# jambo6/online-neural-cdes

Measured on AMD Instinct MI355X. Metric: solved integration steps/sec (fwd+adjoint), higher is better.
Workload: dtype f32; 1 GPU; BASELINE cfg2: rectilinear interpolation, rk4 step 1, B=4096 per GPU (global 4096), raw L=200 -> T=399 knots, C=20, H=HH=32, nl=3; step = forward + adjoint backward + Adam; global_batch=4096, seq_len=200, parallelism=dp1

## Files before the change

### include/ncde_hip.h

```cpp
#ifndef NCDE_HIP_H
#define NCDE_HIP_H

#include <stddef.h>
#include <stdint.h>

#ifdef __cplusplus
extern "C" {
#endif

#define NCDE_ABI_VERSION 4
#define NCDE_MAX_LAYERS 8

typedef enum NcdeStatus {
    NCDE_OK = 0,
    NCDE_ERR_INVALID = -1,
    NCDE_ERR_UNSUPPORTED = -2,
    NCDE_ERR_WORKSPACE = -3,
    NCDE_ERR_HIP = -4
} NcdeStatus;

typedef enum NcdeInterp { NCDE_INTERP_LINEAR = 0, NCDE_INTERP_CUBIC = 1, NCDE_INTERP_QUINTIC = 2 } NcdeInterp;

typedef enum NcdeMethod { NCDE_EULER = 0, NCDE_MIDPOINT = 1, NCDE_RK4_38 = 2 } NcdeMethod;

typedef enum NcdeOutput { NCDE_OUT_INTERVAL = 0, NCDE_OUT_KNOTS = 1, NCDE_OUT_TIMES = 2 } NcdeOutput;

#define NCDE_FLAG_AUTO 0u
#define NCDE_FLAG_FORCE_GENERIC 1u
#define NCDE_FLAG_FORCE_FAST 2u
#define NCDE_FLAG_FP32_MFMA 4u
#define NCDE_FLAG_ADJOINT_V1 8u
#define NCDE_FLAG_ADJOINT_V2 16u
#define NCDE_FLAG_ADJOINT_V4 32u
#define NCDE_FLAG_SPLIT_BF16 64u
#define NCDE_FLAG_ADJOINT_SPLIT_FP16 128u
#define NCDE_FLAG_DEBUG_PROFILE 0x100u
#define NCDE_FLAG_NO_COOP 0x400u
#define NCDE_FLAG_COOP_FAULT_INJECT 0x800u
#define NCDE_FLAG_TILED_NS1 0x1000u
#define NCDE_FLAG_TILED_NS2 0x2000u
#define NCDE_FLAG_TILED_NS4 0x4000u
#define NCDE_FLAG_FORCE_TILED 0x8000u

#define NCDE_FLAG_TILED_WINDOW_STEPS(n) (((uint32_t)(n) & 0xFFu) << 16)

typedef struct NcdeProblem {
    int32_t abi_version;
    int32_t batch;
    int32_t n_knots;
    int32_t channels;
    int32_t hidden;
    int32_t interp;
    int32_t method;
    int32_t output;
    uint32_t flags;

    int32_t n_layers;
    int32_t layer_in[NCDE_MAX_LAYERS];
    int32_t layer_out[NCDE_MAX_LAYERS];
    const float* layer_W[NCDE_MAX_LAYERS];
    const float* layer_b[NCDE_MAX_LAYERS];
    const float* Wo;
    const float* bo;

    const float* coeffs;
    int64_t coeffs_stride_b;
    int64_t coeffs_stride_t;

    const float* z0;

    int32_t field_kind;
    int32_t field_input;
    const float* Wg;
    const float* bg;
    const float* Wr;
    const float* br;

    const void* time_plan;
    int32_t n_t_out;
    int32_t n_steps_fwd;
    int32_t n_steps_adj;
    int32_t reserved_;
} NcdeProblem;

typedef enum NcdeFieldKind { NCDE_FIELD_ORIGINAL = 0, NCDE_FIELD_MINIMAL = 1, NCDE_FIELD_GRU = 2 } NcdeFieldKind;
typedef enum NcdeFieldInput { NCDE_INPUT_MATMUL = 0, NCDE_INPUT_EVALUATE = 1, NCDE_INPUT_DERIVATIVE = 2 } NcdeFieldInput;

typedef struct NcdeGrads {
    float* grad_z0;
    float* grad_layer_W[NCDE_MAX_LAYERS];
    float* grad_layer_b[NCDE_MAX_LAYERS];
    float* grad_Wo;
    float* grad_bo;
    float* grad_Wg;
    float* grad_bg;
    float* grad_Wr;
    float* grad_br;
} NcdeGrads;

typedef struct NcdeTimeSpec {
    int32_t n_t;
    int32_t time_is_f64;
    const double* t;
    double step_size;
    const double* knots;
} NcdeTimeSpec;

typedef struct NcdeTimePlanInfo {
    int32_t n_t_out;
    int32_t n_steps_fwd;
    int32_t n_steps_adj;
    int32_t stages;
    int64_t bytes;
} NcdeTimePlanInfo;

int ncde_time_plan_build(const NcdeProblem* p, const NcdeTimeSpec* ts, void* host_buffer, size_t bytes, NcdeTimePlanInfo* info);

typedef struct NcdeAdaptiveOptions {
    double rtol, atol;
    double min_step;
    double max_step;
    double first_step;
    double safety, ifactor, dfactor;
    int32_t max_num_steps;
    int32_t trace_capacity;
    double* trace;
    int32_t replay_count;
    int32_t reserved_;
    const double* replay;
} NcdeAdaptiveOptions;

typedef struct NcdeAdaptiveStats {
    int32_t nfe;
    int32_t n_accepted, n_rejected;
    int32_t reserved_;
} NcdeAdaptiveStats;

int64_t ncde_dopri5_workspace_bytes(const NcdeProblem* p, const NcdeTimeSpec* ts, int pass );
const char* ncde_dopri5_kernel_name(const NcdeProblem* p, int pass );
int ncde_dopri5_forward(const NcdeProblem* p, const NcdeTimeSpec* ts, const NcdeAdaptiveOptions* opt, float* out, void* workspace,
                        size_t workspace_bytes, void* stream, NcdeAdaptiveStats* stats);
int ncde_dopri5_adjoint(const NcdeProblem* p, const NcdeTimeSpec* ts, const NcdeAdaptiveOptions* opt, const float* z_out,
                        const float* grad_out, const NcdeGrads* grads, void* workspace, size_t workspace_bytes, void* stream,
                        NcdeAdaptiveStats* stats);

int64_t ncde_dopri5_record_bytes(const NcdeProblem* p, const NcdeTimeSpec* ts, const NcdeAdaptiveOptions* opt);
int ncde_dopri5_forward_record(const NcdeProblem* p, const NcdeTimeSpec* ts, const NcdeAdaptiveOptions* opt, float* out, void* record,
                               size_t record_bytes, void* workspace, size_t workspace_bytes, void* stream, NcdeAdaptiveStats* stats);
int ncde_dopri5_backward(const NcdeProblem* p, const NcdeTimeSpec* ts, const NcdeAdaptiveOptions* opt, const void* record,
                         size_t record_bytes, const float* grad_out, const NcdeGrads* grads, void* workspace, size_t workspace_bytes,
                         void* stream);

int ncde_version(void);
const char* ncde_last_error_string(void);

int ncde_num_outputs(const NcdeProblem* p);

int64_t ncde_workspace_bytes(const NcdeProblem* p, int pass);

int64_t ncde_coop_status_offset(const NcdeProblem* p, int pass);

const char* ncde_kernel_name(const NcdeProblem* p, int pass);

int ncde_forward(const NcdeProblem* p, float* out, void* workspace, size_t workspace_bytes, void* stream);

int ncde_adjoint(const NcdeProblem* p, const float* z_out, const float* grad_out, const NcdeGrads* grads,
                 void* workspace, size_t workspace_bytes, void* stream);

int64_t ncde_stage_record_bytes(const NcdeProblem* p);
int ncde_forward_record(const NcdeProblem* p, float* out, float* stages, void* workspace, size_t workspace_bytes, void* stream);
int ncde_backward(const NcdeProblem* p, const float* stages, const float* grad_out, const NcdeGrads* grads, void* workspace,
                  size_t workspace_bytes, void* stream);

int64_t ncde_control_workspace_bytes(const NcdeProblem* p);
const char* ncde_control_kernel_name(const NcdeProblem* p);
int ncde_backward_control(const NcdeProblem* p, const float* stages, const float* grad_out, const NcdeGrads* grads, float* grad_coeffs,
                          void* workspace, size_t workspace_bytes, void* stream);

int ncde_time_kernel(const NcdeProblem* p, int pass, float* out, const float* grad_out, const NcdeGrads* grads,
                     void* workspace, size_t workspace_bytes, void* stream, int iters, float* ms_per_launch);

int64_t ncde_prepare_workspace_bytes(int kind, int B, int L, int C);
int ncde_prepare_linear(const float* x, int B, int L, int C, int rectilinear_time_index, float* out, void* stream);
int ncde_prepare_cubic(const float* x, int B, int L, int C, float* out, void* workspace, size_t workspace_bytes, void* stream);
int ncde_prepare_linear_grid(const float* x, const float* t, int B, int L, int C, int rectilinear_time_index, float* out, void* stream);
int ncde_prepare_cubic_grid(const float* x, const float* t, int B, int L, int C, float* out, void* workspace, size_t workspace_bytes, void* stream);
const char* ncde_prepare_kernel_name(int kind, int B, int L, int C, int has_grid, int rectilinear_time_index);


int ncde_smooth_pieces(int T, double eps);
int ncde_prepare_smooth(const float* x, int B, int T, int C, double eps, int order, float* out, void* stream);

#ifdef __cplusplus
}
#endif
// ... 2 lines not shown
```

### online-neural-cdes_amd/_lib.py

```python
import ctypes
import os

NCDE_ABI_VERSION = 4
NCDE_MAX_LAYERS = 8

INTERP = {"linear": 0, "cubic": 1, "quintic": 2}
INTERP_PARTS = {"linear": 1, "cubic": 4, "quintic": 6}
METHOD = {"euler": 0, "midpoint": 1, "rk4": 2}
OUT_INTERVAL, OUT_KNOTS, OUT_TIMES = 0, 1, 2
FIELD_KIND = {"original": 0, "minimal": 1, "gru": 2}
FIELD_INPUT = {"matmul": 0, "evaluate": 1, "derivative": 2}
FLAG_AUTO, FLAG_FORCE_GENERIC, FLAG_FORCE_FAST, FLAG_FP32_MFMA, FLAG_ADJOINT_V1, FLAG_ADJOINT_V2 = 0, 1, 2, 4, 8, 16
FLAG_ADJOINT_V4 = 32
FLAG_SPLIT_BF16 = 64
FLAG_NO_COOP = 0x400
FLAG_COOP_FAULT_INJECT = 0x800
FLAG_ADJOINT_SPLIT_FP16 = 128


def FLAG_TILED_WINDOW_STEPS(n):
    return (int(n) & 0xFF) << 16
FLAG_TILED_NS1, FLAG_TILED_NS2, FLAG_TILED_NS4, FLAG_FORCE_TILED = 0x1000, 0x2000, 0x4000, 0x8000

_c_float_p = ctypes.c_void_p


class NcdeProblem(ctypes.Structure):
    _fields_ = [
        ("abi_version", ctypes.c_int32),
        ("batch", ctypes.c_int32),
        ("n_knots", ctypes.c_int32),
        ("channels", ctypes.c_int32),
        ("hidden", ctypes.c_int32),
        ("interp", ctypes.c_int32),
        ("method", ctypes.c_int32),
        ("output", ctypes.c_int32),
        ("flags", ctypes.c_uint32),
        ("n_layers", ctypes.c_int32),
        ("layer_in", ctypes.c_int32 * NCDE_MAX_LAYERS),
        ("layer_out", ctypes.c_int32 * NCDE_MAX_LAYERS),
        ("layer_W", _c_float_p * NCDE_MAX_LAYERS),
        ("layer_b", _c_float_p * NCDE_MAX_LAYERS),
        ("Wo", _c_float_p),
        ("bo", _c_float_p),
        ("coeffs", _c_float_p),
        ("coeffs_stride_b", ctypes.c_int64),
        ("coeffs_stride_t", ctypes.c_int64),
        ("z0", _c_float_p),
        ("field_kind", ctypes.c_int32),
        ("field_input", ctypes.c_int32),
        ("Wg", _c_float_p),
        ("bg", _c_float_p),
        ("Wr", _c_float_p),
        ("br", _c_float_p),
        ("time_plan", ctypes.c_void_p),
        ("n_t_out", ctypes.c_int32),
        ("n_steps_fwd", ctypes.c_int32),
        ("n_steps_adj", ctypes.c_int32),
        ("reserved_", ctypes.c_int32),
    ]


class NcdeTimeSpec(ctypes.Structure):
    _fields_ = [
        ("n_t", ctypes.c_int32),
        ("time_is_f64", ctypes.c_int32),
        ("t", ctypes.POINTER(ctypes.c_double)),
        ("step_size", ctypes.c_double),
        ("knots", ctypes.POINTER(ctypes.c_double)),
    ]


class NcdeTimePlanInfo(ctypes.Structure):
    _fields_ = [
        ("n_t_out", ctypes.c_int32),
        ("n_steps_fwd", ctypes.c_int32),
        ("n_steps_adj", ctypes.c_int32),
        ("stages", ctypes.c_int32),
        ("bytes", ctypes.c_int64),
    ]


class NcdeAdaptiveOptions(ctypes.Structure):
    _fields_ = [(n, ctypes.c_double) for n in ("rtol", "atol", "min_step", "max_step", "first_step", "safety", "ifactor", "dfactor")] + \
               [("max_num_steps", ctypes.c_int32), ("trace_capacity", ctypes.c_int32), ("trace", ctypes.POINTER(ctypes.c_double)),
                ("replay_count", ctypes.c_int32), ("reserved_", ctypes.c_int32), ("replay", ctypes.POINTER(ctypes.c_double))]


class NcdeAdaptiveStats(ctypes.Structure):
    _fields_ = [("nfe", ctypes.c_int32), ("n_accepted", ctypes.c_int32), ("n_rejected", ctypes.c_int32), ("reserved_", ctypes.c_int32)]


class NcdeGrads(ctypes.Structure):
    _fields_ = [
        ("grad_z0", _c_float_p),
        ("grad_layer_W", _c_float_p * NCDE_MAX_LAYERS),
        ("grad_layer_b", _c_float_p * NCDE_MAX_LAYERS),
        ("grad_Wo", _c_float_p),
        ("grad_bo", _c_float_p),
        ("grad_Wg", _c_float_p),
        ("grad_bg", _c_float_p),
        ("grad_Wr", _c_float_p),
        ("grad_br", _c_float_p),
    ]


EXPORTS = (
    "ncde_version", "ncde_last_error_string", "ncde_num_outputs", "ncde_workspace_bytes",
    "ncde_kernel_name", "ncde_forward", "ncde_adjoint", "ncde_time_kernel",
    "ncde_prepare_workspace_bytes", "ncde_prepare_linear", "ncde_prepare_cubic", "ncde_prepare_linear_grid", "ncde_prepare_cubic_grid",
    "ncde_prepare_kernel_name",
    "ncde_smooth_pieces", "ncde_prepare_smooth",
    "ncde_stage_record_bytes", "ncde_forward_record", "ncde_backward",
    "ncde_time_plan_build", "ncde_dopri5_workspace_bytes", "ncde_dopri5_forward", "ncde_dopri5_adjoint",
    "ncde_dopri5_record_bytes", "ncde_dopri5_forward_record", "ncde_dopri5_backward", "ncde_dopri5_kernel_name",
    "ncde_coop_status_offset",
    "ncde_control_workspace_bytes", "ncde_control_kernel_name", "ncde_backward_control",
)

_LIB = None
LIB_PATH = os.path.join(os.path.dirname(os.path.abspath(__file__)), "libncde_hip.so")


class NcdeError(RuntimeError):
    pass


def source_fingerprint():
    import glob
    import hashlib
    here = os.path.dirname(os.path.abspath(__file__))
    files = sorted(glob.glob(os.path.join(here, "csrc", "*.hip")) + glob.glob(os.path.join(here, "csrc", "*.h")))
    files.append(os.path.join(os.path.dirname(here), "include", "ncde_hip.h"))
    h = hashlib.sha256()
    for f in files:
        h.update(os.path.basename(f).encode())
        with open(f, "rb") as fh:
            h.update(fh.read())
    return h.hexdigest()


def lib():
    global _LIB
    if _LIB is not None:
        return _LIB
    if not os.path.exists(LIB_PATH):
        raise NcdeError(
            "libncde_hip.so is not built (%s). Run `python __graft_entry__.py` or "
            "`make -C online-neural-cdes_amd/csrc`; there is no CPU fallback." % LIB_PATH)
    h = ctypes.CDLL(LIB_PATH)
    P = ctypes.POINTER(NcdeProblem)
    G = ctypes.POINTER(NcdeGrads)
    vp, sz = ctypes.c_void_p, ctypes.c_size_t
    h.ncde_version.restype = ctypes.c_int
    h.ncde_last_error_string.restype = ctypes.c_char_p
    h.ncde_num_outputs.argtypes = [P]
    h.ncde_num_outputs.restype = ctypes.c_int
    h.ncde_workspace_bytes.argtypes = [P, ctypes.c_int]
    h.ncde_workspace_bytes.restype = ctypes.c_int64
    h.ncde_coop_status_offset.argtypes = [P, ctypes.c_int]
    h.ncde_coop_status_offset.restype = ctypes.c_int64
    h.ncde_kernel_name.argtypes = [P, ctypes.c_int]
    h.ncde_kernel_name.restype = ctypes.c_char_p
    h.ncde_forward.argtypes = [P, vp, vp, sz, vp]
    h.ncde_forward.restype = ctypes.c_int
    h.ncde_adjoint.argtypes = [P, vp, vp, G, vp, sz, vp]
    h.ncde_adjoint.restype = ctypes.c_int
    h.ncde_time_kernel.argtypes = [P, ctypes.c_int, vp, vp, G, vp, sz, vp, ctypes.c_int, ctypes.POINTER(ctypes.c_float)]
    h.ncde_time_kernel.restype = ctypes.c_int
    h.ncde_stage_record_bytes.argtypes = [P]
# ... 61 lines not shown
```

### online-neural-cdes_amd/csrc/ncde_common.h

```cpp
#pragma once
#include <hip/hip_runtime.h>
#include <stdint.h>

#include "ncde_hip.h"

typedef float f32x4 __attribute__((ext_vector_type(4)));

__device__ __forceinline__ float quintic_eval(const float* p, int cs, float f, bool value) {
    const float bb = p[cs], c2 = p[2 * cs], d3 = p[3 * cs], e4 = p[4 * cs], f5 = p[5 * cs];
    if (value) {
        float inner = 0.25f * e4 + (f5 * f) / 5.0f;
        inner = d3 / 3.0f + inner * f;
        inner = 0.5f * c2 + inner * f;
        inner = bb + inner * f;
        return p[0] + inner * f;
    }
    float inner = e4 + f5 * f;
    inner = d3 + inner * f;
    inner = c2 + inner * f;
    return bb + inner * f;
}

#define NCDE_TILE 16

struct KArgs {
    int B, T, C, H, interp, method, output, n_layers, n_pieces, n_out;
    int din[NCDE_MAX_LAYERS], dout[NCDE_MAX_LAYERS];
    const float* W[NCDE_MAX_LAYERS];
    const float* b[NCDE_MAX_LAYERS];
    const float* Wo;
    const float* bo;
    const float* coeffs;
    long long cs_b, cs_t;
    const float* z0;
    float* out;
    const float* z_out;
    const float* grad_out;
    float* grad_z0;
    float* gpart;
    int gW_off[NCDE_MAX_LAYERS], gb_off[NCDE_MAX_LAYERS];
    int gWo_off, gbo_off, theta_size;
    int gacc_in_lds;
    float* stages;
    int discrete;
    float* recA;
    float* recB;
    float* recC;
    float* recD;
    int gstride;
    int win_hi, win_lo, resume;
    float* carry;
    int field_kind, field_input;
    int d0;
    int rows;
    const float* Wg;
    const float* bg;
    const float* Wr;
    const float* br;
    int gWg_off, gbg_off, gWr_off, gbr_off;
    const int* plan;
    int n_steps_fwd, n_steps_adj;
    const float* Wo_pk;
    int* fault;
    int only_faulted;
    const float* Wg_pk;
    const unsigned* Wo_bf;
    int wres[NCDE_MAX_LAYERS], wres_o, wres_g, wres_r;
    int tres[NCDE_MAX_LAYERS], tres_o, tres_g;
    int Hr, Cc;
    const unsigned* coop_img;
    float* coop_x;
    float* coop_state;
    unsigned* coop_sync;
    const float* coop_scale;
    int coop_M, coop_G;
    float* recS;
    unsigned* win_max;
    int dw2_parts;
    int dw2_accum;
    int Brec;
    unsigned* coop_status;
    const unsigned* run_if;
    unsigned coop_spin;
    int coop_inject;
};

typedef void (*NcdeKernel)(KArgs);

#define NCDE_PLAN_MAGIC 0x4e43504c
#define NCDE_PLAN_HEADER 8
struct StageDesc {
    int idx;
    float frac;
    float kdt;
};
__host__ __device__ __forceinline__ int plan_step_words(int S) { return 3 + 3 * S; }
__host__ __device__ __forceinline__ int plan_off_fwd() { return NCDE_PLAN_HEADER; }
__host__ __device__ __forceinline__ int plan_off_out(int S, int n_fwd) { return NCDE_PLAN_HEADER + n_fwd * plan_step_words(S); }
__host__ __device__ __forceinline__ int plan_off_adj(int S, int n_fwd, int n_out) { return plan_off_out(S, n_fwd) + 2 * n_out; }
__device__ __forceinline__ bool plan_header_ok(const KArgs& a, int S) {
    const int* h = a.plan;
    return h[0] == NCDE_PLAN_MAGIC && h[1] == S && h[2] == a.n_steps_fwd && h[3] == a.n_steps_adj && h[4] == a.n_out;
}
__device__ __forceinline__ StageDesc plan_stage(const int* step, int j) {
    StageDesc d;
    d.idx = step[3 + 3 * j];
    d.frac = __int_as_float(step[4 + 3 * j]);
    d.kdt = __int_as_float(step[5 + 3 * j]);
    return d;
}

__device__ __forceinline__ int ru4(int x) { return (x + 3) & ~3; }
__device__ __forceinline__ int ru16(int x) { return (x + 15) & ~15; }

__device__ __forceinline__ f32x4 mfma16(float a, float b, f32x4 c) {
    return __builtin_amdgcn_mfma_f32_16x16x4f32(a, b, c, 0, 0, 0);
}

__device__ __forceinline__ float tanh_dev(float x) {
    const float e = __builtin_amdgcn_exp2f(x * 2.8853900817779268f);
    const float r = __builtin_amdgcn_rcpf(e + 1.0f);
    return __builtin_fmaf(-2.0f, r, 1.0f);
}

#define NCDE_TANH_PRESCALE 2.8853900817779268f
__device__ __forceinline__ float tanh_prescaled(float x2l) {
    const float e = __builtin_amdgcn_exp2f(x2l);
    const float r = __builtin_amdgcn_rcpf(e + 1.0f);
    return __builtin_fmaf(-2.0f, r, 1.0f);
}

__device__ __forceinline__ float relu_dev(float x) { return __builtin_amdgcn_fmed3f(x, 0.0f, __builtin_inff()); }

__device__ __forceinline__ int n_stages(int method) { return method == NCDE_RK4_38 ? 4 : (method == NCDE_MIDPOINT ? 2 : 1); }
__device__ __forceinline__ float stage_offset(int method, int j) {
    if (method == NCDE_RK4_38) return j == 0 ? 0.0f : (j == 1 ? 0.333333343267440796f : (j == 2 ? 0.666666686534881592f : 1.0f));
    if (method == NCDE_MIDPOINT) return j == 0 ? 0.0f : 0.5f;
    return 0.0f;
}
__device__ __forceinline__ float stage_weight(int method, int j) {
    if (method == NCDE_RK4_38) return (j == 0 || j == 3) ? 0.125f : 0.375f;
    if (method == NCDE_MIDPOINT) return j == 0 ? 0.0f : 1.0f;
    return 1.0f;
}

__device__ __forceinline__ int piece_index(float t, int n_pieces) {
    int idx = (int)__builtin_ceilf(t) - 1;
    idx = idx < 0 ? 0 : idx;
    return idx > n_pieces - 1 ? n_pieces - 1 : idx;
}

__device__ __forceinline__ float row16_sum(float v) {
    v += __shfl_xor(v, 8, 64);
    v += __shfl_xor(v, 4, 64);
    v += __shfl_xor(v, 2, 64);
    v += __shfl_xor(v, 1, 64);
    return v;
}

struct StageCombine {
    __device__ static __forceinline__ float apply(int method, int j, float k, float dt, float& y0, float& k1, float& k2, bool& last) {
        last = false;
        if (method == NCDE_RK4_38) {
            if (j == 0) { k1 = k; return y0 + (dt * k) * 0.333333343267440796f; }
            if (j == 1) { k2 = k; return y0 + dt * (k - k1 * 0.333333343267440796f); }
            if (j == 2) { const float ys = y0 + dt * ((k1 - k2) + k); k2 = k2 + k; return ys; }
            last = true;
            y0 = y0 + (((k1 + 3.0f * k2) + k) * dt) * 0.125f;
            return y0;
        }
        if (method == NCDE_MIDPOINT) {
            if (j == 0) return y0 + k * (0.5f * dt);
            last = true;
            y0 = y0 + dt * k;
            return y0;
        }
        last = true;
        y0 = y0 + dt * k;
        return y0;
    }
};

__device__ __forceinline__ StageDesc default_stage(int method, float t, int n_pieces) {
    StageDesc d;
    d.idx = piece_index(t, n_pieces);
    d.frac = t - (float)d.idx;
    d.kdt = 1.0f;
    return d;
}

__device__ __forceinline__ float plan_out_cotangent(const KArgs& a, const int* pstep, const int* pout, int part, long long brow, int h) {
    float acc = 0.0f;
    const int q0 = pstep[1], q1 = q0 + pstep[2];
    for (int q = q0; q < q1; ++q) {
        const int kind = pout[2 * q];
        const float slope = __int_as_float(pout[2 * q + 1]);
        const float g = a.grad_out[(brow + q) * a.Hr + h];
        if (part == 1) acc += kind == 1 ? g : (kind == 2 ? slope * g : 0.0f);
        else acc += kind == 0 ? g : (kind == 2 ? g - slope * g : 0.0f);
    }
    return acc;
}
```

### online-neural-cdes_amd/csrc/ncde_fast.hip

```cpp
#include "ncde_fast.h"
#include "ncde_fast4.h"
#include "ncde_fast64.h"
#include "ncde_fast_nl.h"
#include "ncde_fast_c.h"
#include "ncde_fast_fwd3.h"
#include "ncde_fast_plan.h"
#ifndef NCDE_F2_DW_LATE
#define NCDE_F2_DW_LATE 0
#endif
#ifndef NCDE_F2_DXL_BF3
#define NCDE_F2_DXL_BF3 1
#endif
#ifndef NCDE_F2_DWO_EARLY
#define NCDE_F2_DWO_EARLY 0
#endif
#ifndef NCDE_H2_DW_LATE
#define NCDE_H2_DW_LATE 1
#endif
#ifndef NCDE_H2_DWO_EARLY
#define NCDE_H2_DWO_EARLY 0
#endif

#include <cstring>
#include <type_traits>
// ... 115 lines not shown

    const int n_inner = a.n_layers - 1;
    int zpar = 0;
    if constexpr (PROF != 0) tlast = __builtin_readcyclecounter();
    for (int n = 0; n < a.T - 1; ++n) {
        if (n + 1 < a.n_pieces) stage_load(n + 1);
#pragma unroll
        for (int j = 0; j < S; ++j) {
            const float t = (float)n + stage_offset(METHOD, j);
            const int idx = piece_index(t, a.n_pieces);
            const float frac = t - (float)idx;
            const float* dxp = dxs[idx % 3] + s * DXW;
            if (a.stages != nullptr && wave == ((n * S + j) % NW) && valid) {
                float* rec = a.stages + ((long long)(n * S + j) * a.B + bs) * a.Hr;
#pragma unroll
                for (int ks = 0; ks < HB; ++ks)
                    if (4 * ks + g < a.Hr) rec[4 * ks + g] = zreg[ks];
            }
            f32x4 acc[HT];
            float hB[KH];
#pragma unroll
            for (int tt = 0; tt < HT; ++tt) acc[tt] = bias0[tt];
#pragma unroll
            for (int ks = 0; ks < HB; ++ks)
#pragma unroll
                for (int tt = 0; tt < HT; ++tt) acc[tt] = mfma16(w0[tt][ks], zreg[ks], acc[tt]);
#pragma unroll
            for (int tt = 0; tt < HT; ++tt)
#pragma unroll
                for (int r = 0; r < 4; ++r) hB[4 * tt + r] = relu_dev(acc[tt][r]);
            for (int rep = 0; rep < n_inner; ++rep) {
#pragma unroll
                for (int tt = 0; tt < HT; ++tt) acc[tt] = bias1[tt];
#pragma unroll
                for (int ks = 0; ks < KH; ++ks)
#pragma unroll
                    for (int tt = 0; tt < HT; ++tt) acc[tt] = mfma16(w1[tt][ks], hB[ks], acc[tt]);
#pragma unroll
                for (int tt = 0; tt < HT; ++tt)
#pragma unroll
                    for (int r = 0; r < 4; ++r) hB[4 * tt + r] = relu_dev(acc[tt][r]);
            }
            NCDE_TICK(0)
            float kout[NB];
#pragma unroll
            for (int nb = 0; nb < NB; ++nb) kout[nb] = 0.0f;
            f32x4 oprev[NB];
#pragma unroll
            for (int cq = 0; cq <= CQ; ++cq) {
                f32x4 o[NB];
                if (cq < CQ) {
#pragma unroll
                    for (int nb = 0; nb < NB; ++nb) o[nb] = biaso[nb][cq];
#pragma unroll
                    for (int ks = 0; ks < KH; ++ks)
#pragma unroll
                        for (int nb = 0; nb < NB; ++nb) o[nb] = mfma16(wo[nb][cq][ks], hB[ks], o[nb]);
                }
                if (cq > 0) {
                    const int cp = cq - 1;
                    f32x4 dx;
                    if constexpr (INTERP == NCDE_INTERP_LINEAR) {
                        dx = *reinterpret_cast<const f32x4*>(dxp + 4 * cp);
                    } else {
                        const f32x4 cb = *reinterpret_cast<const f32x4*>(dxp + 4 * cp);
                        const f32x4 cc = *reinterpret_cast<const f32x4*>(dxp + CP + 4 * cp);
                        const f32x4 cd = *reinterpret_cast<const f32x4*>(dxp + 2 * CP + 4 * cp);
#pragma unroll
                        for (int r = 0; r < 4; ++r) {
                            const float inner = cc[r] + cd[r] * frac;
                            dx[r] = cb[r] + inner * frac;
                        }
                    }
#pragma unroll
                    for (int nb = 0; nb < NB; ++nb)
#pragma unroll
                        for (int r = 0; r < 4; ++r) kout[nb] = fmaf(tanh_prescaled(oprev[nb][r]), dx[r], kout[nb]);
                }
                if (cq > 0 && cq < CQ) {
#pragma unroll
                    for (int i = 0; i < KH * NB; ++i) {
                        __builtin_amdgcn_sched_group_barrier(0x008, 1, 0);
                        __builtin_amdgcn_sched_group_barrier(0x002, 3, 0);
                    }
                }
#pragma unroll
                for (int nb = 0; nb < NB; ++nb) oprev[nb] = o[nb];
            }
            NCDE_TICK(1)
            float ys[NB];
#pragma unroll
            for (int nb = 0; nb < NB; ++nb) ys[nb] = Combine<METHOD>::apply(j, kout[nb], y0[nb], k1[nb], k2[nb]);
            if (j == S - 1) {
                if (valid && (a.output == NCDE_OUT_KNOTS || n == a.T - 2)) {
                    const int row = a.output == NCDE_OUT_KNOTS ? n + 1 : 1;
#pragma unroll
                    for (int nb = 0; nb < NB; ++nb)
                        if (4 * (wave * NB + nb) + g < a.Hr) a.out[((long long)bs * a.n_out + row) * a.Hr + 4 * (wave * NB + nb) + g] = ys[nb];
                }
                if (n + 1 < a.n_pieces) stage_store(n + 1);
            }
            if constexpr (NW == 1) {
#pragma unroll
                for (int nb = 0; nb < NB; ++nb) zreg[nb] = ys[nb];
                __builtin_amdgcn_fence(__ATOMIC_RELEASE, "wavefront");
            } else {
                float* zw = zx[zpar];
#pragma unroll
                for (int nb = 0; nb < NB; ++nb) zw[(4 * (wave * NB + nb) + g) * 16 + s] = ys[nb];
                __syncthreads();
#pragma unroll
                for (int ks = 0; ks < HB; ++ks) zreg[ks] = zw[(4 * ks + g) * 16 + s];
                zpar ^= 1;
            }
            NCDE_TICK(2)
        }
    }
    if constexpr (PROF != 0) {
        if (lane == 0) {
            unsigned long long* dst = reinterpret_cast<unsigned long long*>(a.gpart) + ((long long)blockIdx.x * NW + wave) * 4;
            dst[0] = prof[0]; dst[1] = prof[1]; dst[2] = prof[2]; dst[3] = prof[3];
        }
    }
#undef NCDE_TICK
}

template <int H, int HH, int C, int NW, int INTERP, int METHOD, int PROF = 0, int NLT = 0, int HP = 0, int PLAN = 0>
__global__ __launch_bounds__(64 * NW, (NW + 3) / 4) void ncde_fwd_fast_bf3(KArgs a) {
    unsigned long long prof[4] = {0, 0, 0, 0}, tlast = 0;
#define NCDE_TICK(k)                                                \
    if constexpr (PROF != 0) {                                      \
        const unsigned long long now_ = __builtin_readcyclecounter(); \
        prof[k] += now_ - tlast;                                    \
        tlast = now_;                                               \
    }
    constexpr int CP = (C + 3) & ~3, CQ = CP / 4, HB = H / 4, HT = HH / 16, NB = HB / NW;
    constexpr int KC0 = H / 32, KC = HH / 32;
    constexpr int S = kStages<METHOD>;
    constexpr int NT = 64 * NW;
    constexpr int DXW = INTERP == NCDE_INTERP_LINEAR ? CP : 3 * CP;
    constexpr int EPT = (16 * DXW + NT - 1) / NT;
    static_assert(H % (4 * NW) == 0 && HH % 32 == 0 && H % 32 == 0, "shape not tileable");
    __shared__ __attribute__((aligned(16))) float zx[2][H * 16];
    __shared__ __attribute__((aligned(16))) float dxs[PLAN ? 1 : 3][PLAN ? 4 : 16 * DXW];
    __shared__ __attribute__((aligned(16))) float dxq[PLAN ? 2 : 1][PLAN ? S * 16 * CP : 4];
    __shared__ int fault_s;
    if constexpr (HP == 0) {
        if (a.only_faulted && a.fault[blockIdx.x] == 0) return;
    }
    if constexpr (PLAN != 0) {
        if (a.plan == nullptr || !plan_header_ok(a, S)) return;
    }
    float mx = 0.0f;

    const int tid = threadIdx.x, lane = tid & 63;
    const int wave = __builtin_amdgcn_readfirstlane(tid >> 6);
    const int s = lane & 15, g = lane >> 4;
    const int b0 = blockIdx.x * NCDE_TILE;
    const int bs = b0 + s;
    const bool valid = bs < a.B;

    typedef SplitOps<HP> SO;
    typedef typename SO::T SpT;
    SpT w0[HT][KC0], w1[HT][KC], wo[NB][CQ][KC];
    f32x4 bias0[HT], bias1[HT], biaso[NB][CQ];
    const bool has_inner = a.n_layers > 1;
#pragma unroll
    for (int t = 0; t < HT; ++t) {
        const int unitA = 32 * (t >> 1) + 8 * (s >> 2) + 4 * (t & 1) + (s & 3);
        float tmp[8];
#pragma unroll
        for (int c = 0; c < KC0; ++c) {
#pragma unroll
            for (int j = 0; j < 8; ++j) tmp[j] = a.W[0][unitA * H + 32 * c + 8 * g + j];
            w0[t][c] = SO::split(tmp, mx);
        }
#pragma unroll
        for (int c = 0; c < KC; ++c) {
#pragma unroll
            for (int j = 0; j < 8; ++j) tmp[j] = has_inner ? a.W[1][unitA * HH + 32 * c + 8 * g + j] : 0.0f;
            w1[t][c] = SO::split(tmp, mx);
        }
#pragma unroll
        for (int r = 0; r < 4; ++r) {
            const int unitD = 32 * (t >> 1) + 8 * g + 4 * (t & 1) + r;
            bias0[t][r] = a.b[0][unitD];
            bias1[t][r] = has_inner ? a.b[1][unitD] : 0.0f;
        }
    }
#pragma unroll
    for (int nb = 0; nb < NB; ++nb) {
        const int hb = wave * NB + nb;
#pragma unroll
        for (int cq = 0; cq < CQ; ++cq) {
            const int hA = 4 * hb + (s >> 2), cA = 4 * cq + (s & 3);
            float tmp[8];
#pragma unroll
            for (int c = 0; c < KC; ++c) {
#pragma unroll
                for (int j = 0; j < 8; ++j) tmp[j] = cA < C ? NCDE_TANH_PRESCALE * a.Wo[(hA * C + cA) * HH + 32 * c + 8 * g + j] : 0.0f;
                wo[nb][cq][c] = SO::split(tmp, mx);
            }
#pragma unroll
            for (int r = 0; r < 4; ++r) {
                const int cc = 4 * cq + r;
                biaso[nb][cq][r] = cc < C ? NCDE_TANH_PRESCALE * a.bo[(4 * hb + g) * C + cc] : 0.0f;
            }
        }
    }

    const float* eptr[EPT];
    float eprev[EPT], enext[EPT];
    bool eok[EPT];
#pragma unroll
    for (int q = 0; q < EPT; ++q) {
        const int e = tid + q * NT;
        const int es = e / DXW, ec = e - es * DXW;
        const int part = ec / CP, c = ec - part * CP;
        eok[q] = e < 16 * DXW && c < a.Cc && (b0 + es) < a.B;
        const long long base = (long long)(eok[q] ? b0 + es : 0) * a.cs_b;
        eptr[q] = a.coeffs + base + (INTERP == NCDE_INTERP_LINEAR ? c : (part + 1) * a.Cc + c);
        eprev[q] = 0.0f;
        enext[q] = 0.0f;
    }
    auto stage_load = [&](int piece) {
#pragma unroll
        for (int q = 0; q < EPT; ++q) {
            const int row = INTERP == NCDE_INTERP_LINEAR ? piece + 1 : piece;
            enext[q] = eok[q] ? eptr[q][(long long)row * a.cs_t] : 0.0f;
        }
    };
    auto stage_store = [&](int piece) {
        float* dst = dxs[piece % 3];
#pragma unroll
        for (int q = 0; q < EPT; ++q) {
            const int e = tid + q * NT;
            if (e < 16 * DXW) dst[e] = INTERP == NCDE_INTERP_LINEAR ? enext[q] - eprev[q] : enext[q];
            eprev[q] = enext[q];
        }
    };
    constexpr int EPQ = PLAN ? (S * 16 * CP + NT - 1) / NT : 1;
    float qn[EPQ];
    auto plan_load = [&](const int* pstep) {
#pragma unroll
        for (int q = 0; q < EPQ; ++q) {
            const int e = tid + q * NT;
            const int j = e / (16 * CP), rem = e - j * (16 * CP), es = rem / CP, c = rem - es * CP;
            float v = 0.0f;
            if (e < S * 16 * CP && c < a.Cc && b0 + es < a.B) {
                const StageDesc sd = plan_stage(pstep, j);
                const float* p = a.coeffs + (long long)(b0 + es) * a.cs_b + (long long)sd.idx * a.cs_t;
                if constexpr (INTERP == NCDE_INTERP_LINEAR) {
                    v = p[a.cs_t + c] - p[c];
                    if (sd.kdt != 1.0f) v = v / sd.kdt;
                } else {
                    const float bb = p[a.Cc + c], cc = p[2 * a.Cc + c], dd = p[3 * a.Cc + c];
                    const float inner = cc + dd * sd.frac;
                    v = bb + inner * sd.frac;
                }
            }
            qn[q] = v;
        }
    };
    auto plan_store = [&](int buf) {
#pragma unroll
        for (int q = 0; q < EPQ; ++q) {
            const int e = tid + q * NT;
            if (e < S * 16 * CP) dxq[buf][e] = qn[q];
        }
    };
    const int pw_ = plan_step_words(S);
    const int* pfwd = PLAN ? a.plan + plan_off_fwd() : nullptr;
    const int* pout = PLAN ? a.plan + plan_off_out(S, a.n_steps_fwd) : nullptr;
    const int n_steps = PLAN ? a.n_steps_fwd : a.T - 1;
    if constexpr (PLAN != 0) {
        plan_load(pfwd);
        plan_store(0);
    } else {
        if (INTERP == NCDE_INTERP_LINEAR) {
#pragma unroll
            for (int q = 0; q < EPT; ++q) eprev[q] = eok[q] ? eptr[q][0] : 0.0f;
        }
        stage_load(0);
        stage_store(0);
    }

    float y0[NB], k1[NB], k2[NB], zreg[KC0][8];
#pragma unroll
    for (int c = 0; c < KC0; ++c)
#pragma unroll
        for (int j = 0; j < 8; ++j) zreg[c][j] = (valid && 32 * c + 8 * g + j < a.Hr) ? a.z0[(long long)bs * a.Hr + 32 * c + 8 * g + j] : 0.0f;
#pragma unroll
    for (int nb = 0; nb < NB; ++nb) {
        const int u = 4 * (wave * NB + nb) + g;
        y0[nb] = (valid && u < a.Hr) ? a.z0[(long long)bs * a.Hr + u] : 0.0f;
        k1[nb] = 0.0f;
        k2[nb] = 0.0f;
        if (valid && u < a.Hr) a.out[((long long)bs * a.n_out) * a.Hr + u] = y0[nb];
    }
    __syncthreads();

    const int n_inner = a.n_layers - 1;
    int zpar = 0;
    if constexpr (PROF != 0) tlast = __builtin_readcyclecounter();
    for (int n = 0; n < n_steps; ++n) {
        const int* pstep = PLAN ? pfwd + n * pw_ : nullptr;
        const float dt = PLAN ? __int_as_float(pstep[0]) : 1.0f;
        if constexpr (PLAN != 0) {
            if (n + 1 < n_steps) plan_load(pstep + pw_);
        } else {
            if (n + 1 < a.n_pieces) stage_load(n + 1);
        }
#pragma unroll
        for (int j = 0; j < S; ++j) {
            const float t = (float)n + stage_offset(METHOD, j);
            const int idx = PLAN ? 0 : piece_index(t, a.n_pieces);
            const float frac = t - (float)idx;
            const float* dxp = PLAN ? dxq[n & 1] + (j * 16 + s) * CP : dxs[idx % 3] + s * DXW;
            if (a.stages != nullptr && wave == ((n * S + j) % NW) && valid) {
                float* rec = a.stages + ((long long)(n * S + j) * a.B + bs) * a.Hr;
                if (a.Hr == H) {
#pragma unroll
                    for (int c = 0; c < KC0; ++c) {
                        *reinterpret_cast<f32x4*>(rec + 32 * c + 8 * g) = (f32x4){zreg[c][0], zreg[c][1], zreg[c][2], zreg[c][3]};
                        *reinterpret_cast<f32x4*>(rec + 32 * c + 8 * g + 4) = (f32x4){zreg[c][4], zreg[c][5], zreg[c][6], zreg[c][7]};
                    }
                } else {
#pragma unroll
                    for (int c = 0; c < KC0; ++c)
#pragma unroll
                        for (int jj = 0; jj < 8; ++jj)
                            if (32 * c + 8 * g + jj < a.Hr) rec[32 * c + 8 * g + jj] = zreg[c][jj];
                }
            }
            typename SO::Acc acc[HT];
            float hv[KC][8];
            SpT xb[KC];
            auto activate = [&]() {
#pragma unroll
                for (int tt = 0; tt < HT; ++tt) {
                    const f32x4 pre = SO::finish(acc[tt]);
#pragma unroll
                    for (int r = 0; r < 4; ++r) hv[tt >> 1][4 * (tt & 1) + r] = relu_bits(pre[r]);
                }
#pragma unroll
                for (int c = 0; c < KC; ++c) xb[c] = SO::split(hv[c], mx);
            };
            {
                SpT zb[KC0];
#pragma unroll
                for (int c = 0; c < KC0; ++c) zb[c] = SO::split(zreg[c], mx);
#pragma unroll
                for (int tt = 0; tt < HT; ++tt) acc[tt] = SO::init(bias0[tt]);
#pragma unroll
                for (int c = 0; c < KC0; ++c)
#pragma unroll
                    for (int tt = 0; tt < HT; ++tt) SO::mac(w0[tt][c], zb[c], acc[tt]);
            }
            activate();
            auto inner_layer = [&]() {
#pragma unroll
                for (int tt = 0; tt < HT; ++tt) acc[tt] = SO::init(bias1[tt]);
#pragma unroll
                for (int c = 0; c < KC; ++c)
#pragma unroll
                    for (int tt = 0; tt < HT; ++tt) SO::mac(w1[tt][c], xb[c], acc[tt]);
                activate();
            };
            if constexpr (NLT > 0) {
#pragma unroll
                for (int rep = 0; rep < NLT - 1; ++rep) inner_layer();
            } else {
                for (int rep = 0; rep < n_inner; ++rep) inner_layer();
            }
            NCDE_TICK(0)
            float kout[NB];
#pragma unroll
            for (int nb = 0; nb < NB; ++nb) kout[nb] = 0.0f;
#pragma unroll
            for (int cq = 0; cq < CQ; ++cq) {
                typename SO::Acc oa[NB];
                f32x4 o[NB];
#pragma unroll
                for (int nb = 0; nb < NB; ++nb) oa[nb] = SO::init(biaso[nb][cq]);
#pragma unroll
                for (int c = 0; c < KC; ++c)
#pragma unroll
                    for (int nb = 0; nb < NB; ++nb) SO::mac(wo[nb][cq][c], xb[c], oa[nb]);
#pragma unroll
                for (int nb = 0; nb < NB; ++nb) o[nb] = SO::finish(oa[nb]);
                f32x4 dx;
                if constexpr (INTERP == NCDE_INTERP_LINEAR || PLAN != 0) {
                    dx = *reinterpret_cast<const f32x4*>(dxp + 4 * cq);
                } else {
                    const f32x4 cb = *reinterpret_cast<const f32x4*>(dxp + 4 * cq);
                    const f32x4 cc = *reinterpret_cast<const f32x4*>(dxp + CP + 4 * cq);
                    const f32x4 cd = *reinterpret_cast<const f32x4*>(dxp + 2 * CP + 4 * cq);
#pragma unroll
                    for (int r = 0; r < 4; ++r) {
                        const float inner = cc[r] + cd[r] * frac;
                        dx[r] = cb[r] + inner * frac;
                    }
                }
#pragma unroll
                for (int nb = 0; nb < NB; ++nb)
#pragma unroll
                    for (int r = 0; r < 4; ++r) kout[nb] = fmaf(tanh_prescaled(o[nb][r]), dx[r], kout[nb]);
            }
            NCDE_TICK(1)
            float ys[NB], yprev[NB];
#pragma unroll
            for (int nb = 0; nb < NB; ++nb) {
                yprev[nb] = y0[nb];
                if constexpr (PLAN != 0) {
                    bool last;
                    ys[nb] = StageCombine::apply(METHOD, j, kout[nb], dt, y0[nb], k1[nb], k2[nb], last);
                } else {
                    ys[nb] = Combine<METHOD>::apply(j, kout[nb], y0[nb], k1[nb], k2[nb]);
                }
            }
            if (j == S - 1) {
                if constexpr (PLAN != 0) {
                    if (valid) {
                        const int q0 = pstep[1], q1 = q0 + pstep[2];
                        for (int r = q0; r < q1; ++r) {
                            const int kind = pout[2 * r];
                            const float slope = __int_as_float(pout[2 * r + 1]);
#pragma unroll
                            for (int nb = 0; nb < NB; ++nb)
                                if (4 * (wave * NB + nb) + g < a.Hr)
                                    a.out[((long long)bs * a.n_out + r) * a.Hr + 4 * (wave * NB + nb) + g] =
                                        kind == 1 ? ys[nb] : (kind == 0 ? yprev[nb] : yprev[nb] + slope * (ys[nb] - yprev[nb]));
                        }
                    }
                    if (n + 1 < n_steps) plan_store((n + 1) & 1);
                } else {
                    if (valid && (a.output == NCDE_OUT_KNOTS || n == a.T - 2)) {
                        const int row = a.output == NCDE_OUT_KNOTS ? n + 1 : 1;
#pragma unroll
                        for (int nb = 0; nb < NB; ++nb)
                            if (4 * (wave * NB + nb) + g < a.Hr) a.out[((long long)bs * a.n_out + row) * a.Hr + 4 * (wave * NB + nb) + g] = ys[nb];
                    }
                    if (n + 1 < a.n_pieces) stage_store(n + 1);
                }
            }
            {
                float* zw = zx[zpar];
#pragma unroll
                for (int nb = 0; nb < NB; ++nb) zw[(4 * (wave * NB + nb) + g) * 16 + s] = ys[nb];
                __syncthreads();
#pragma unroll
                for (int c = 0; c < KC0; ++c)
#pragma unroll
                    for (int jj = 0; jj < 8; ++jj) zreg[c][jj] = zw[(32 * c + 8 * g + jj) * 16 + s];
                zpar ^= 1;
            }
            NCDE_TICK(2)
        }
    }
    if constexpr (PROF != 0) {
        if (lane == 0) {
            unsigned long long* dst = reinterpret_cast<unsigned long long*>(a.gpart) + ((long long)blockIdx.x * NW + wave) * 4;
            dst[0] = prof[0]; dst[1] = prof[1]; dst[2] = prof[2]; dst[3] = prof[3];
        }
    }
    if constexpr (HP != 0) {
        if (a.fault != nullptr) {
            if (tid == 0) fault_s = 0;
            __syncthreads();
            if (__builtin_amdgcn_ballot_w64(h2_range_fault(mx)) != 0 && lane == 0) fault_s = 1;
            __syncthreads();
            if (tid == 0) a.fault[blockIdx.x] = fault_s;
        }
    }
#undef NCDE_TICK
}

template <int H, int HH, int C, int NL, int NW, int INTERP, int METHOD, int PROF = 0>
__global__ __launch_bounds__(64 * NW, 1) void ncde_adj_fast(KArgs a) {
    unsigned long long prof[6] = {0, 0, 0, 0, 0, 0}, tlast = 0;
#define NCDE_TICK(k)                                                \
    if constexpr (PROF != 0) {                                      \
        const unsigned long long now_ = __builtin_readcyclecounter(); \
        prof[k] += now_ - tlast;                                    \
        tlast = now_;                                               \
    }
    constexpr int CP = (C + 3) & ~3, CQ = CP / 4, HB = H / 4, HT = HH / 16, KH = HH / 4, NB = HB / NW;
    constexpr int S = kStages<METHOD>;
    constexpr int NT = 64 * NW;
    constexpr int DXW = INTERP == NCDE_INTERP_LINEAR ? CP : 3 * CP;
    constexpr int EPT = (16 * DXW + NT - 1) / NT;
    constexpr int NTILE = NB * CQ;
    constexpr int HT0 = H / 16;
    constexpr int TPW1 = HT * HT / NW, TPW0 = HT * HT0 / NW;
    constexpr int XS = 20;
    constexpr int IMG = (H + NL * HH) * XS;
    constexpr int PRIV = IMG + HH * XS;
    static_assert(H % (4 * NW) == 0 && HH % 16 == 0 && H % 16 == 0 && NB <= 4, "shape not tileable");
    static_assert((HT * HT) % NW == 0 && (HT * HT0) % NW == 0, "weight-gradient tiles must split evenly over the waves");
    extern __shared__ __attribute__((aligned(16))) float lds[];
    float* zx = lds;
    float* dxs = zx + 2 * H * 16;
    float* red = dxs + 3 * 16 * DXW;
    float* woT = red + NW * HH * 16;
    float* boL = woT + NW * NTILE * HT * 256;
    float* privbase = boL + NW * NTILE * 16;

    const int tid = threadIdx.x, lane = tid & 63;
    const int wave = __builtin_amdgcn_readfirstlane(tid >> 6);
    const int s = lane & 15, g = lane >> 4;
    const int b0 = blockIdx.x * NCDE_TILE;
    const int bs = b0 + s;
    const bool valid = bs < a.B;
    float* priv = privbase + wave * PRIV;
    float* img = priv;
    float* dpimg = priv + IMG;
    float* dptile = dpimg;
    const float* woTw = woT + wave * NTILE * HT * 256;
    const float* boLw = boL + wave * NTILE * 16;

    float w0[HT][HB], w1[HT][KH], wo[NB][CQ][KH], w1T[HT][KH], w0T[KH];
    f32x4 bias0[HT], bias1[HT];
#pragma unroll
    for (int t = 0; t < HT; ++t) {
        const int unitA = 4 * (4 * t + (s & 3)) + (s >> 2);
#pragma unroll
        for (int ks = 0; ks < HB; ++ks) w0[t][ks] = a.W[0][unitA * H + 4 * ks + g];
#pragma unroll
        for (int ks = 0; ks < KH; ++ks) {
            w1[t][ks] = a.W[1][unitA * HH + 4 * ks + g];
            w1T[t][ks] = a.W[1][(4 * ks + g) * HH + unitA];
        }
#pragma unroll
        for (int r = 0; r < 4; ++r) {
            const int unitD = 4 * (4 * t + r) + g;
            bias0[t][r] = a.b[0][unitD];
            bias1[t][r] = a.b[1][unitD];
        }
    }
    {
        const int r_own = s & 3;
        const int hrow = 4 * (wave * NB + r_own) + (s >> 2);
#pragma unroll
        for (int ks = 0; ks < KH; ++ks) w0T[ks] = r_own < NB ? a.W[0][(4 * ks + g) * H + hrow] : 0.0f;
    }
#pragma unroll
    for (int nb = 0; nb < NB; ++nb) {
        const int hb = wave * NB + nb;
#pragma unroll
        for (int cq = 0; cq < CQ; ++cq) {
            const int hA = 4 * hb + (s >> 2), cA = 4 * cq + (s & 3);
#pragma unroll
            for (int ks = 0; ks < KH; ++ks) wo[nb][cq][ks] = cA < C ? NCDE_TANH_PRESCALE * a.Wo[(hA * C + cA) * HH + 4 * ks + g] : 0.0f;
        }
    }
    for (int e = tid; e < NW * NTILE * HT * 256; e += NT) {
        const int r = e & 3, l = (e >> 2) & 63, rest = e >> 8;
        const int tp = rest % HT, tau = (rest / HT) % NTILE, wv = rest / (HT * NTILE);
        const int nb = tau / CQ, cq = tau - nb * CQ;
        const int h = 4 * (wv * NB + nb) + (l >> 4), c = 4 * cq + r;
        const int jrow = 4 * (4 * tp + (l & 3)) + ((l & 15) >> 2);
        woT[e] = c < C ? a.Wo[(h * C + c) * HH + jrow] : 0.0f;
    }
    for (int e = tid; e < NW * NTILE * 16; e += NT) {
        const int r = e & 3, gg = (e >> 2) & 3, rest = e >> 4;
        const int tau = rest % NTILE, wv = rest / NTILE;
        const int nb = tau / CQ, cq = tau - nb * CQ;
        const int h = 4 * (wv * NB + nb) + gg, c = 4 * cq + r;
        boL[e] = c < C ? NCDE_TANH_PRESCALE * a.bo[h * C + c] : 0.0f;
    }

    const float* eptr[EPT];
    float eprev[EPT], enext[EPT];
    bool eok[EPT];
#pragma unroll
    for (int q = 0; q < EPT; ++q) {
        const int e = tid + q * NT;
        const int es = e / DXW, ec = e - es * DXW;
        const int part = ec / CP, c = ec - part * CP;
        eok[q] = e < 16 * DXW && c < a.Cc && (b0 + es) < a.B;
        const long long base = (long long)(eok[q] ? b0 + es : 0) * a.cs_b;
        eptr[q] = a.coeffs + base + (INTERP == NCDE_INTERP_LINEAR ? c : (part + 1) * a.Cc + c);
        eprev[q] = 0.0f;
        enext[q] = 0.0f;
    }
    auto stage_load = [&](int piece) {
#pragma unroll
        for (int q = 0; q < EPT; ++q) enext[q] = eok[q] ? eptr[q][(long long)piece * a.cs_t] : 0.0f;
    };
    auto stage_store = [&](int piece) {
        float* dst = dxs + (piece % 3) * 16 * DXW;
#pragma unroll
        for (int q = 0; q < EPT; ++q) {
            const int e = tid + q * NT;
            if (e < 16 * DXW) dst[e] = INTERP == NCDE_INTERP_LINEAR ? eprev[q] - enext[q] : enext[q];
            eprev[q] = enext[q];
        }
    };
    const int p_hi = a.n_pieces - 1;
    if (INTERP == NCDE_INTERP_LINEAR) {
#pragma unroll
        for (int q = 0; q < EPT; ++q) eprev[q] = eok[q] ? eptr[q][(long long)(p_hi + 1) * a.cs_t] : 0.0f;
    }
    stage_load(p_hi);
    stage_store(p_hi);
    if (p_hi >= 1) {
        stage_load(p_hi - 1);
        stage_store(p_hi - 1);
// ... 2098 lines not shown
```

### online-neural-cdes_amd/csrc/ncde_host.h

```cpp
#pragma once
#include <mutex>
#include <map>
#include <utility>
#include <hip/hip_runtime.h>

#include <algorithm>
#include <cstring>

#include "ncde_common.h"

struct ReduceSegs {
    int n;
    int off[2 * NCDE_MAX_LAYERS + 6];
    int len[2 * NCDE_MAX_LAYERS + 6];
    float* dst[2 * NCDE_MAX_LAYERS + 6];
};
extern "C" __global__ void ncde_reduce_partials(const float* gpart, int n_part, int theta_size, ReduceSegs segs);

constexpr int kLdsLimit = 160 * 1024;

constexpr uint32_t kFlagChainDump = 0x200u;

inline const char* ncde_dev_env(const char* name) {
#ifdef NCDE_DEV_KNOBS
    return getenv(name);
#else
    (void)name;
    return nullptr;
#endif
}

inline hipError_t ncde_lds_optin(const void* fn, size_t bytes) {
    static std::mutex mu;
    static std::map<std::pair<int, const void*>, size_t> granted;
    int dev = 0;
    if (hipGetDevice(&dev) != hipSuccess) dev = 0;
    std::lock_guard<std::mutex> lk(mu);
    size_t& have = granted[{dev, fn}];
    if (bytes <= have) return hipSuccess;
    const hipError_t e = hipFuncSetAttribute(fn, hipFuncAttributeMaxDynamicSharedMemorySize, (int)bytes);
    if (e == hipSuccess) have = bytes;
    return e;
}
inline int hru4(int x) { return (x + 3) & ~3; }
inline int hru16(int x) { return (x + 15) & ~15; }

struct Layout {
    int Hp, Cp, Dp, HS, DS, L;
    int theta_size;
    int gW_off[NCDE_MAX_LAYERS], gb_off[NCDE_MAX_LAYERS], gWo_off, gbo_off;
    int gWg_off, gbg_off, gWr_off, gbr_off;
    int d0, rows;
    bool variant;
    int dlast;
    int n_wg;
    size_t lds_fwd, lds_adj;
    int gacc_in_lds;
};

inline Layout make_layout(const NcdeProblem* p) {
    Layout y{};
    y.L = p->n_layers;
    y.Hp = hru16(p->hidden);
    y.Cp = hru4(p->channels);
    y.variant = p->field_kind != NCDE_FIELD_ORIGINAL || p->field_input != NCDE_INPUT_MATMUL;
    y.d0 = p->field_input == NCDE_INPUT_MATMUL ? p->hidden : p->hidden + p->channels;
    y.rows = p->field_input == NCDE_INPUT_MATMUL ? p->hidden * p->channels : p->hidden;
    y.Dp = std::max(y.Hp, hru16(y.d0));
    for (int l = 0; l < y.L; ++l) y.Dp = std::max(y.Dp, hru16(p->layer_out[l]));
    y.HS = y.Hp * 16;
    y.DS = y.Dp * 16;
    y.dlast = y.L ? p->layer_out[y.L - 1] : p->hidden;
    int off = 0;
    for (int l = 0; l < y.L; ++l) {
        int prevW = -1, prevB = -1;
        for (int q = 0; q < l; ++q) {
            if (p->layer_W[q] == p->layer_W[l]) prevW = q;
            if (p->layer_b[q] == p->layer_b[l]) prevB = q;
        }
        if (prevW >= 0) y.gW_off[l] = y.gW_off[prevW];
        else { y.gW_off[l] = off; off += p->layer_out[l] * p->layer_in[l]; }
        if (prevB >= 0) y.gb_off[l] = y.gb_off[prevB];
        else { y.gb_off[l] = off; off += p->layer_out[l]; }
    }
    y.gWo_off = off; off += y.rows * y.dlast;
    y.gbo_off = off; off += y.rows;
    y.gWg_off = y.gbg_off = y.gWr_off = y.gbr_off = 0;
    if (p->field_kind != NCDE_FIELD_ORIGINAL) {
        y.gWg_off = off; off += y.rows * y.dlast;
        y.gbg_off = off; off += y.rows;
    }
    if (p->field_kind == NCDE_FIELD_GRU) {
        y.gWr_off = off; off += y.d0 * y.d0;
        y.gbr_off = off; off += y.d0;
    }
    y.theta_size = off;
    y.n_wg = (p->batch + NCDE_TILE - 1) / NCDE_TILE;
    y.lds_fwd = sizeof(float) * (size_t)(5 * y.HS + 2 * y.DS + y.Cp * 16);
    size_t adj = sizeof(float) * (size_t)(10 * y.HS + ((y.L > 0 ? y.L : 1) + 4) * y.DS + y.Cp * 16 + 4 * 16 * 17);
    y.gacc_in_lds = adj + sizeof(float) * (size_t)y.theta_size <= (size_t)kLdsLimit;
    y.lds_adj = adj + (y.gacc_in_lds ? sizeof(float) * (size_t)y.theta_size : 0);
    return y;
}


inline void fill_kargs(const NcdeProblem* p, const Layout& y, KArgs* a) {
    memset(a, 0, sizeof(*a));
    a->B = p->batch; a->T = p->n_knots; a->C = p->channels; a->H = p->hidden;
    a->interp = p->interp; a->method = p->method; a->output = p->output; a->n_layers = p->n_layers;
    a->n_pieces = p->n_knots - 1;
    a->n_out = p->output == NCDE_OUT_TIMES ? p->n_t_out : (p->output == NCDE_OUT_KNOTS ? p->n_knots : 2);
    if (p->output == NCDE_OUT_TIMES) {
        a->plan = (const int*)p->time_plan;
        a->n_steps_fwd = p->n_steps_fwd;
        a->n_steps_adj = p->n_steps_adj;
    }
    for (int l = 0; l < p->n_layers; ++l) {
        a->din[l] = p->layer_in[l]; a->dout[l] = p->layer_out[l];
        a->W[l] = p->layer_W[l]; a->b[l] = p->layer_b[l];
        a->gW_off[l] = y.gW_off[l]; a->gb_off[l] = y.gb_off[l];
    }
    a->Wo = p->Wo; a->bo = p->bo; a->coeffs = p->coeffs;
    a->cs_b = p->coeffs_stride_b; a->cs_t = p->coeffs_stride_t;
    a->z0 = p->z0;
    a->gWo_off = y.gWo_off; a->gbo_off = y.gbo_off; a->theta_size = y.theta_size;
    a->field_kind = p->field_kind; a->field_input = p->field_input; a->d0 = y.d0; a->rows = y.rows;
    a->Wg = p->Wg; a->bg = p->bg; a->Wr = p->Wr; a->br = p->br;
    a->gWg_off = y.gWg_off; a->gbg_off = y.gbg_off; a->gWr_off = y.gWr_off; a->gbr_off = y.gbr_off;
    a->gacc_in_lds = y.gacc_in_lds;
    a->Hr = p->reserved_ ? (p->reserved_ >> 12) : p->hidden;
    a->Cc = p->reserved_ ? (p->reserved_ & 0xFFF) : p->channels;
}

inline int launch_reduce_partials(const NcdeProblem* p, const Layout& y, const NcdeGrads* g, const float* gpart, int n_part,
                                  hipStream_t st) {
    ReduceSegs segs{};
    int n = 0;
    for (int l = 0; l < p->n_layers; ++l) {
        bool firstW = true, firstB = true;
        for (int q = 0; q < l; ++q) {
            if (p->layer_W[q] == p->layer_W[l]) firstW = false;
            if (p->layer_b[q] == p->layer_b[l]) firstB = false;
        }
        if (firstW) { segs.off[n] = y.gW_off[l]; segs.len[n] = p->layer_out[l] * p->layer_in[l]; segs.dst[n] = g->grad_layer_W[l]; ++n; }
        if (firstB) { segs.off[n] = y.gb_off[l]; segs.len[n] = p->layer_out[l]; segs.dst[n] = g->grad_layer_b[l]; ++n; }
    }
    segs.off[n] = y.gWo_off; segs.len[n] = y.rows * y.dlast; segs.dst[n] = g->grad_Wo; ++n;
    segs.off[n] = y.gbo_off; segs.len[n] = y.rows; segs.dst[n] = g->grad_bo; ++n;
    if (p->field_kind != NCDE_FIELD_ORIGINAL) {
        segs.off[n] = y.gWg_off; segs.len[n] = y.rows * y.dlast; segs.dst[n] = g->grad_Wg; ++n;
        segs.off[n] = y.gbg_off; segs.len[n] = y.rows; segs.dst[n] = g->grad_bg; ++n;
    }
    if (p->field_kind == NCDE_FIELD_GRU) {
        segs.off[n] = y.gWr_off; segs.len[n] = y.d0 * y.d0; segs.dst[n] = g->grad_Wr; ++n;
        segs.off[n] = y.gbr_off; segs.len[n] = y.d0; segs.dst[n] = g->grad_br; ++n;
    }
    segs.n = n;
    for (int i = 0; i < n; ++i)
        if (!segs.dst[i]) return NCDE_ERR_INVALID;
    hipLaunchKernelGGL(ncde_reduce_partials, dim3((y.theta_size + 255) / 256), dim3(256), 0, st, gpart, n_part, y.theta_size, segs);
    return hipGetLastError() == hipSuccess ? NCDE_OK : NCDE_ERR_HIP;
}
```

Before: 177.0 million sample-steps/s.

## Skip output-projection blocks whose control increments are all zero in forward

```diff
diff --git a/include/ncde_hip.h b/include/ncde_hip.h
--- a/include/ncde_hip.h
+++ b/include/ncde_hip.h
@@ -41,6 +41,7 @@
 #define NCDE_FLAG_TILED_NS2 0x2000u
 #define NCDE_FLAG_TILED_NS4 0x4000u
 #define NCDE_FLAG_FORCE_TILED 0x8000u
+#define NCDE_FLAG_NO_ZERO_SKIP 0x1000000u
 
 #define NCDE_FLAG_TILED_WINDOW_STEPS(n) (((uint32_t)(n) & 0xFFu) << 16)
 
diff --git a/online-neural-cdes_amd/_lib.py b/online-neural-cdes_amd/_lib.py
--- a/online-neural-cdes_amd/_lib.py
+++ b/online-neural-cdes_amd/_lib.py
@@ -16,6 +16,7 @@
 FLAG_NO_COOP = 0x400
 FLAG_COOP_FAULT_INJECT = 0x800
 FLAG_ADJOINT_SPLIT_FP16 = 128
+FLAG_NO_ZERO_SKIP = 0x1000000
 
 
 def FLAG_TILED_WINDOW_STEPS(n):
diff --git a/online-neural-cdes_amd/csrc/ncde_common.h b/online-neural-cdes_amd/csrc/ncde_common.h
--- a/online-neural-cdes_amd/csrc/ncde_common.h
+++ b/online-neural-cdes_amd/csrc/ncde_common.h
@@ -83,6 +83,7 @@
     const unsigned* run_if;
     unsigned coop_spin;
     int coop_inject;
+    int no_zero_skip;
 };
 
 typedef void (*NcdeKernel)(KArgs);
diff --git a/online-neural-cdes_amd/csrc/ncde_fast.hip b/online-neural-cdes_amd/csrc/ncde_fast.hip
--- a/online-neural-cdes_amd/csrc/ncde_fast.hip
+++ b/online-neural-cdes_amd/csrc/ncde_fast.hip
@@ -291,6 +291,10 @@
         if (a.plan == nullptr || !plan_header_ok(a, S)) return;
     }
     float mx = 0.0f;
+    constexpr bool ZSKIP = HP != 0 && INTERP == NCDE_INTERP_LINEAR && PLAN == 0;
+    constexpr unsigned ZFULL = (1u << CQ) - 1u;
+    static_assert(3 * CQ <= 32, "one mask of CQ bits per ring slot in one word");
+    bool wnan = false;
 
     const int tid = threadIdx.x, lane = tid & 63;
     const int wave = __builtin_amdgcn_readfirstlane(tid >> 6);
@@ -338,6 +342,10 @@
             for (int c = 0; c < KC; ++c) {
 #pragma unroll
                 for (int j = 0; j < 8; ++j) tmp[j] = cA < C ? NCDE_TANH_PRESCALE * a.Wo[(hA * C + cA) * HH + 32 * c + 8 * g + j] : 0.0f;
+                if constexpr (ZSKIP) {
+#pragma unroll
+                    for (int j = 0; j < 8; j += 2) wnan |= __builtin_isunordered(tmp[j], tmp[j + 1]);
+                }
                 wo[nb][cq][c] = SO::split(tmp, mx);
             }
 #pragma unroll
@@ -345,8 +353,10 @@
                 const int cc = 4 * cq + r;
                 biaso[nb][cq][r] = cc < C ? NCDE_TANH_PRESCALE * a.bo[(4 * hb + g) * C + cc] : 0.0f;
             }
-        }
-    }
+            if constexpr (ZSKIP) wnan |= __builtin_isunordered(biaso[nb][cq][0], biaso[nb][cq][1]) | __builtin_isunordered(biaso[nb][cq][2], biaso[nb][cq][3]);
+        }
+    }
+    const bool zforce = ZSKIP && (a.no_zero_skip != 0 || __builtin_amdgcn_ballot_w64(wnan) != 0);
 
     const float* eptr[EPT];
     float eprev[EPT], enext[EPT];
@@ -438,6 +448,21 @@
         if (valid && u < a.Hr) a.out[((long long)bs * a.n_out) * a.Hr + u] = y0[nb];
     }
     __syncthreads();
+    auto slot_mask = [&](int slot) -> unsigned {
+        const float* row = dxs[PLAN ? 0 : slot] + s * DXW;
+        unsigned m = 0;
+#pragma unroll
+        for (int cq = 0; cq < CQ; ++cq) {
+            const f32x4 d = *reinterpret_cast<const f32x4*>(row + 4 * cq);
+            const bool nz = (d[0] != 0.0f) | (d[1] != 0.0f) | (d[2] != 0.0f) | (d[3] != 0.0f);
+            m |= __builtin_amdgcn_ballot_w64(nz) != 0 ? 1u << cq : 0u;
+        }
+        return __builtin_amdgcn_readfirstlane(m);
+    };
+    unsigned zmask = 0;
+    if constexpr (ZSKIP) {
+        if (!zforce) zmask = slot_mask(0);
+    }
 
     const int n_inner = a.n_layers - 1;
     int zpar = 0;
@@ -516,8 +541,8 @@
             float kout[NB];
 #pragma unroll
             for (int nb = 0; nb < NB; ++nb) kout[nb] = 0.0f;
-#pragma unroll
-            for (int cq = 0; cq < CQ; ++cq) {
+            auto out_block = [&](auto cq_c) {
+                constexpr int cq = decltype(cq_c)::value;
                 typename SO::Acc oa[NB];
                 f32x4 o[NB];
 #pragma unroll
@@ -545,6 +570,36 @@
                 for (int nb = 0; nb < NB; ++nb)
 #pragma unroll
                     for (int r = 0; r < 4; ++r) kout[nb] = fmaf(tanh_prescaled(o[nb][r]), dx[r], kout[nb]);
+            };
+            auto out_blocks = [&](auto skip_c, unsigned m) {
+                auto one = [&](auto cq_c) {
+                    constexpr int cq = decltype(cq_c)::value;
+                    if constexpr (cq < CQ) {
+                        if constexpr (decltype(skip_c)::value) {
+                            if ((m >> cq) & 1u) out_block(cq_c);
+                        } else {
+                            out_block(cq_c);
+                        }
+                    }
+                };
+                one(std::integral_constant<int, 0>{}); one(std::integral_constant<int, 1>{}); one(std::integral_constant<int, 2>{});
+                one(std::integral_constant<int, 3>{}); one(std::integral_constant<int, 4>{}); one(std::integral_constant<int, 5>{});
+                one(std::integral_constant<int, 6>{}); one(std::integral_constant<int, 7>{}); one(std::integral_constant<int, 8>{});
+                one(std::integral_constant<int, 9>{});
+                static_assert(CQ <= 10, "extend the block list");
+            };
+            if constexpr (ZSKIP) {
+                bool xnan = false;
+#pragma unroll
+                for (int c = 0; c < KC; ++c)
+#pragma unroll
+                    for (int jj = 0; jj < 8; jj += 2) xnan |= __builtin_isunordered(hv[c][jj], hv[c][jj + 1]);
+                unsigned m = (zmask >> (CQ * (idx % 3))) & ZFULL;
+                if (zforce || __builtin_amdgcn_ballot_w64(xnan) != 0) m = ZFULL;
+                if (m == ZFULL) out_blocks(std::false_type{}, m);
+                else out_blocks(std::true_type{}, m);
+            } else {
+                out_blocks(std::false_type{}, 0u);
             }
             NCDE_TICK(1)
             float ys[NB], yprev[NB];
@@ -593,6 +648,12 @@
 #pragma unroll
                     for (int jj = 0; jj < 8; ++jj) zreg[c][jj] = zw[(32 * c + 8 * g + jj) * 16 + s];
                 zpar ^= 1;
+            }
+            if constexpr (ZSKIP) {
+                if (j == S - 1 && n + 1 < a.n_pieces && !zforce) {
+                    const int sh = CQ * ((n + 1) % 3);
+                    zmask = (zmask & ~(ZFULL << sh)) | (slot_mask((n + 1) % 3) << sh);
+                }
             }
             NCDE_TICK(2)
         }
diff --git a/online-neural-cdes_amd/csrc/ncde_host.h b/online-neural-cdes_amd/csrc/ncde_host.h
--- a/online-neural-cdes_amd/csrc/ncde_host.h
+++ b/online-neural-cdes_amd/csrc/ncde_host.h
@@ -130,6 +130,7 @@
     a->gacc_in_lds = y.gacc_in_lds;
     a->Hr = p->reserved_ ? (p->reserved_ >> 12) : p->hidden;
     a->Cc = p->reserved_ ? (p->reserved_ & 0xFFF) : p->channels;
+    a->no_zero_skip = (p->flags & NCDE_FLAG_NO_ZERO_SKIP) != 0;
 }
 
 inline int launch_reduce_partials(const NcdeProblem* p, const Layout& y, const NcdeGrads* g, const float* gpart, int n_part,
```

Result: no change. 176.9 million sample-steps/s (-0.1%).
